# msracver/Relation-Networks-for-Object-Detection

Measured on AMD Instinct MI355X. Metric: images/sec (1000x600, 300 ROIs), higher is better.
Workload: dtype bf16

## Files before the change

include/relnet_hip.h:

```cpp
#ifndef RELNET_HIP_H
#define RELNET_HIP_H

#ifdef __cplusplus
extern "C" {
#endif

enum { RELNET_F32 = 0, RELNET_BF16 = 1 };

int relnet_version(void);
const char* relnet_last_error(void);
unsigned long long relnet_stream_capture_id(void* stream);

void _nms(int* keep_out, int* num_out, const float* boxes_host, int boxes_num, int boxes_dim,
          float nms_overlap_thresh, int device_id);

int relnet_proposal_decode(const float* cls_prob, const long* cls_strides4, const float* deltas,
                           const long* delta_strides4, const float* im_info, const double* base_anchors,
                           float* boxes , float* scores , int B, int A, int h, int w,
                           int feat_stride, int min_size, int softmax_pairs, void* stream);
int relnet_topk_sort(const float* scores, const float* boxes, float* out_boxes5, int* out_index,
                     int* out_count, int B, int n, int K, void* stream);
int relnet_nms_mask(const float* boxes5, const int* counts , unsigned long long* mask,
                    int B, int n, int n_stride, float thresh, void* stream);
int relnet_nms_scan(const unsigned long long* mask, const float* boxes5, const int* counts, float* rois,
// ... 73 lines not shown

int relnet_geometry_bias(const float* boxes, int box_stride, int box_off, const float* wp_t, const float* bp,
                         const float* divisors8, void* bias, int bias_half , float* pos_mat,
                         float* pos_emb, int B, int N, int M, int Mpad, int fc_dim, int nmod, void* stream);

int relnet_relation_attention(const void* q, long q_ld, long q_bs, const void* k, long k_ld, long k_bs,
                              const void* vwt, long vwt_ld, long vwt_bs, const void* bias, int bias_half,
                              long bias_bs, const float* bout, const void* resid, long resid_ld, long resid_bs, void* out,
                              long out_ld, long out_bs, void* out_act, long act_ld, long act_bs, float* logits,
                              int B, int H, int N, int M, int Mpad, float scale, int in_dtype, int out_dtype,
                              void* stream);

int relnet_relation_attention_kc(const void* q, long q_ld, long q_bs, const void* k, long k_ld, long k_bs,
                                 const void* vwt, long vwt_ld, long vwt_bs, const void* bias, int bias_half,
                                 long bias_bs, const float* bout, const void* resid, long resid_ld, long resid_bs, void* out,
                                 long out_ld, long out_bs, void* out_act, long act_ld, long act_bs, float* logits,
                                 int B, int H, int N, int M, int Mpad, float scale, int in_dtype, int out_dtype,
                                 const int* key_count, void* stream);
void relnet_relation_attention_debug_lds_f32(int on);

int relnet_relation_attention_fused(const void* q, long q_ld, long q_bs, const void* k, long k_ld, long k_bs,
                                    const void* vwt, long vwt_ld, long vwt_bs, const float* boxes, int box_stride,
                                    int box_off, const float* wp, const float* bp, const float* divisors8,
                                    const float* bout, const void* resid, long resid_ld, long resid_bs, void* out,
                                    long out_ld, long out_bs, void* out_act, long act_ld, long act_bs, int B, int H,
                                    int N, int M, int Mpad, float scale, void* stream);

int relnet_bottleneck_chain(const void* mid2, const void* x, const void* w3f, const void* w1f, const float* b3,
                            const float* b1, void* x_next, void* mid1_next, long P, int mid, void* stream);
int relnet_bottleneck_chain_proj(const void* mid2, const void* x_in, const void* w3f, const void* wpf, const void* w1f,
                                 const float* b3p, const float* b1, void* x_next, void* mid1_next, long P, int mid, void* stream);
int relnet_bottleneck_chain_s2(const void* mid2, const void* x, const void* w3f, const float* b3, void* x_next, int B, int H,
                               int W, int mid, void* stream);

int relnet_conv3x3_c64(const void* in, const void* w_frag, const float* bias, int relu, void* out, int B, int H, int W,
                       void* stream);
int relnet_conv3x3_c64_s2(const void* in, const void* w_frag, const float* bias, int relu, void* out, int B, int H, int W,
                          void* stream);


int relnet_pack_w_frag(const void* w, long ldw, void* out, int N, int K, void* stream);
int relnet_conv2d_nhwc_wf(const void* in, long in_pix, long in_img, const void* w, const void* w_frag, const float* bias,
                          const void* resid, int relu, void* out, long ldc, int B, int H, int W, int Cin, int Cout, int R,
                          int S, int stride, int dil, int pad, int out_dtype, void* stream);

int relnet_detect_head(const float* cls_score, long cs_ld, const float* bbox_pred, long bp_ld, const float* rois,
                       const float* im_info, float* cls_prob, double* boxes, int R, int C, int rois_per_image,
                       int delta_off, void* stream);
int relnet_detect_head_ex(const float* cls_score, long cs_ld, const float* bbox_pred, long bp_ld, const float* rois,
                          const float* im_info, float* cls_prob, double* boxes, int R, int C, int rois_per_image,
                          int delta_off, const int* n_valid, void* stream);
int relnet_class_nms(const float* cls_prob, const double* boxes, double* dets, int* counts, int B, int N, int C,
                     float score_thresh, double nms_param, int soft, int max_picks, void* stream);
int relnet_class_nms_ex(const float* cls_prob, const double* scores64, const double* boxes, double* dets, int* counts,
                        int* pick_index, int B, int N, int C, float score_thresh, double nms_param, int soft,
                        int max_picks, void* stream);
int relnet_class_nms_hist_bins(void);
int relnet_class_nms_topk(const float* cls_prob, const double* boxes, double* dets, int* counts, void* hist, int B, int N, int C,
                          float score_thresh, double nms_param, int soft, int max_picks, int top_k, void* stream);
int relnet_image_topk(const double* dets, const int* counts, double* thresh, int* total, float* out,
                      int* out_count, int B, int NC, int N, int max_per_image, int max_out, void* stream);

int relnet_lnms_prepare(const float* cls_score, long cs_ld, const float* bbox_pred, long bp_ld, const float* rois,
                        const float* im_info, float* prob , float* boxes , int B, int N,
                        int C, int delta_off, const float* means4, const float* stds4, void* stream);
int relnet_lnms_prepare_ex(const float* cls_score, long cs_ld, const float* bbox_pred, long bp_ld, const float* rois,
// ... 214 lines not shown
```

relation-networks-for-object-detection_amd/backbone.py:

```python
import math
import os

import torch
import torch.nn.functional as F

from . import ops

UNITS = (3, 4, 23, 3)
FILTERS = (256, 512, 1024, 2048)
EPS = 1e-5
PIXEL_MEANS = (103.06, 115.90, 123.15)


def unit_names(fpn=False):
    out = []
    in_ch = 64
    for si, (n, oc) in enumerate(zip(UNITS, FILTERS)):
        stage = si + 2
        for u in range(n):
            if n <= 3 or stage == 2 or stage == 5:
                name = 'abc'[u]
            else:
                name = 'a' if u == 0 else 'b%d' % u
            stride = 2 if (u == 0 and (stage in (3, 4) or (fpn and stage == 5))) else 1
# ... 51 lines not shown
        p['res5%s_branch2b_offset_weight' % u] = nrm(dcn_offset_std, 72, 512, 3, 3)
        p['res5%s_branch2b_offset_bias' % u] = torch.zeros(72)
    p['offset_weight'] = nrm(dcn_offset_std, 98, 256 * 49); p['offset_bias'] = torch.zeros(98)
    if fpn:
        for lvl, cin in ((32, 2048), (16, 1024), (8, 512), (4, 256)):
            p['fpn_ft%d_1x1_weight' % lvl] = nrm(0.01, 256, cin, 1, 1); p['fpn_ft%d_1x1_bias' % lvl] = torch.zeros(256)
            p['fpn_ft%d_3x3_weight' % lvl] = nrm(0.01, 256, 256, 3, 3); p['fpn_ft%d_3x3_bias' % lvl] = torch.zeros(256)
        p['fpn_ft64_3x3_weight'] = nrm(0.01, 256, 256, 3, 3); p['fpn_ft64_3x3_bias'] = torch.zeros(256)
        p['roi_pool_fc1_weight'] = nrm(0.01, 1024, 256 * 49); p['roi_pool_fc1_bias'] = torch.zeros(1024)
        p['roi_pool_fc2_weight'] = nrm(0.01, 1024, 1024); p['roi_pool_fc2_bias'] = torch.zeros(1024)
    return p


def fold_bn(w, gamma, beta, mean, var, eps=EPS):
    s = gamma.double() / torch.sqrt(var.double() + eps)
    return (w.double() * s.view(-1, 1, 1, 1)).float(), (beta.double() - mean.double() * s).float()


class Backbone(object):

    def __init__(self, params, dtype=torch.bfloat16, device='cuda', channels_last=True, impl=None, stem='hip', dcn=False,
                 fpn=False, chain=True, frozen_only=False, pixel_means=PIXEL_MEANS):
        self.dtype, self.device, self.dcn, self.fpn = dtype, device, dcn, fpn
        self.frozen_only = frozen_only
        self.pixel_means = tuple(float(v) for v in pixel_means)
        self.use_chain = chain
        env = os.environ.get('RELNET_STAGE_SPLIT')
        if env not in (None, '', '0'):
            self.stage_split = {int(a): int(b) for a, b in (kv.split(':') for kv in env.split(','))}
        if os.environ.get('RELNET_INPLACE_EXPAND') is not None:
            self.inplace_expand = os.environ['RELNET_INPLACE_EXPAND'] not in ('', '0')
        if os.environ.get('RELNET_QUARTER_UNITS') is not None:
            self.quarter_units = os.environ['RELNET_QUARTER_UNITS'] not in ('', '0')
        self.impl = impl or ('hip' if dtype == torch.bfloat16 else ('hip32' if dtype == torch.float32 and torch.device(device).type == 'cuda' else 'miopen'))
        if self.impl == 'hip' and torch.device(device).type == 'cuda':
            ops.asm_selfcheck()
        self.stem = stem
        assert self.impl in ('hip', 'hip32', 'miopen') and (self.impl != 'hip' or dtype == torch.bfloat16) and (self.impl != 'hip32' or dtype == torch.float32)
        self.mf = torch.channels_last if channels_last else torch.contiguous_format
        self.w = {}
        self.wp = {}
        self.wf = {}
        self.b32 = {}
        self.wp32 = {}
        for conv, bn, oc, ic, k in conv_bn_names():
            if frozen_only and not conv.startswith(('conv1', 'res2')):
                continue
            w, b = fold_bn(params[conv + '_weight'], params[bn + '_gamma'], params[bn + '_beta'],
                           params[bn + '_moving_mean'], params[bn + '_moving_var'])
            self._put(conv, w, b)
        if frozen_only:
            pass
        elif fpn:
            for lvl in (32, 16, 8, 4):
                for k in ('1x1', '3x3'):
                    name = 'fpn_ft%d_%s' % (lvl, k)
                    self._put(name, params[name + '_weight'], params[name + '_bias'])
        else:
            for name in ('rpn_conv_3x3', 'rpn_cls_score', 'rpn_bbox_pred', 'conv_new_1'):
                self._put(name, params[name + '_weight'], params[name + '_bias'])
            self._put('rpn_out', torch.cat([params['rpn_cls_score_weight'], params['rpn_bbox_pred_weight']], 0),
                      torch.cat([params['rpn_cls_score_bias'], params['rpn_bbox_pred_bias']], 0))
        self.units = [u for u in unit_names(fpn) if not frozen_only or u[0] == 2]
        self.wp_dcn = {}
        if dcn and not frozen_only:
            for u in 'abc':
                name = 'res5%s_branch2b' % u
                self._put(name + '_offset', params[name + '_offset_weight'], params[name + '_offset_bias'])
                w, b = fold_bn(params[name + '_weight'], params['bn5%s_branch2b_gamma' % u], params['bn5%s_branch2b_beta' % u],
                               params['bn5%s_branch2b_moving_mean' % u], params['bn5%s_branch2b_moving_var' % u])
                self.wp_dcn[name] = (ops.pack_conv_weight(w, self.dtype, self.device), b.to(self.device, torch.float32).contiguous())
        if self.impl == 'hip':
            w1, b1 = fold_bn(params['conv1_weight'], params['bn_conv1_gamma'], params['bn_conv1_beta'],
                             params['bn_conv1_moving_mean'], params['bn_conv1_moving_var'])
            self.w_stem = ops.pack_stem_weight(w1, self.dtype, self.device)
            self.zero_bias64 = torch.zeros(64, device=self.device, dtype=torch.float32)
        self.chain, self.halo3, self.chain_proj = {}, {}, {}
        if self.impl == 'hip' and chain:
            reduce_mids = tuple(m for m in ops.CHAIN_MIDS if m != 256 or os.environ.get('RELNET_CHAIN_REDUCE256', '1') != '0')
            for (st, nm, ic, mc, oc, stride, dil, proj), nxt in zip(self.units, self.units[1:] + [None]):
                if nxt is not None and nxt[0] == st and not nxt[7] and mc in reduce_mids:
                    w3, b3, _ = self.wp['res%s_branch2c' % nm]
                    w1n, b1n, _ = self.wp['res%s_branch2a' % nxt[1]]
                    self.chain[nm] = (ops.pack_w_frag(w3), ops.pack_chain_w1(w1n), b3, b1n)
                elif mc in ops.CHAIN_EXPAND_MIDS:
                    w3, b3, _ = self.wp['res%s_branch2c' % nm]
                    self.chain[nm] = (ops.pack_w_frag(w3), None, b3, None)
            for (st, nm, ic, mc, oc, stride, dil, proj) in self.units:
                if proj and stride == 1 and mc == 64 and ic == 64 and nm in self.chain:
                    w3f, w1f, b3, b1n = self.chain[nm]
                    wp_, bp_, _ = self.wp['res%s_branch1' % nm]
                    self.chain_proj[nm] = (w3f, ops.pack_w_frag(wp_), w1f, (b3 + bp_).contiguous(), b1n)
            for st, nm, ic, mc, oc, stride, dil, proj in self.units:
                if mc in ops.HALO3_CHANNELS and dil == 1 and not (self.dcn and st == 5):
                    w, b, _ = self.wp['res%s_branch2b' % nm]
                    self.halo3['res%s_branch2b' % nm] = (ops.pack_w_frag(w, panel_only=False), b)

    def _put(self, name, w, b):
        self.w[name] = (w.to(self.device, self.dtype).contiguous(memory_format=self.mf),
                        b.to(self.device, self.dtype))
        if self.impl == 'hip':
            self.b32[name] = b.to(self.device, torch.float32).contiguous()
        if self.impl == 'hip32':
            if w.shape[1] % 16:
                wz = torch.zeros((w.shape[0], (w.shape[1] + 15) // 16 * 16) + tuple(w.shape[2:]), dtype=w.dtype)
                wz[:, :w.shape[1]] = w
                w = wz
            self.wp32[name] = (ops.pack_conv_weight(w, torch.float32, self.device), b.to(self.device, torch.float32).contiguous(), int(w.shape[2]))
        if self.impl == 'hip' and w.shape[1] % 64 == 0:
            self.wp[name] = (ops.pack_conv_weight(w, self.dtype, self.device),
                             b.to(self.device, torch.float32).contiguous(), int(w.shape[2]))
            if self.dtype == torch.bfloat16 and tuple(w.shape[1:]) == (256, 1, 1) and w.shape[0] % 256 == 0 \
                    and name.endswith('_branch2c'):
                self.wf[name] = ops.pack_w_frag(self.wp[name][0])

    def _hconv(self, x, name, stride=1, pad=0, dil=1, relu=False, resid=None, out_dtype=None):
        w, b, k = self.wp[name]
        return ops.conv2d_nhwc(x, w, b, ksize=k, stride=stride, pad=pad, dil=dil, relu=relu, resid=resid,
                               out_dtype=out_dtype, w_frag=self.wf.get(name))

    def _float_image(self, data, im_info, dtype):
        if data.dtype != torch.uint8:
            return data
        return ops.image_transform_u8(data, self.pixel_means, im_info, dtype=dtype)

    def forward_res2(self, data, im_info=None):
        if self.impl == 'hip32':
            assert self.frozen_only
            return self._forward_hip32(self._float_image(data, im_info, torch.float32))
        x = ops.stem_fused(data, self.w_stem, self.b32['conv1'], im_info, self.pixel_means)
        y_next = None
        self.last_chain_units = []
        for unit in self.units:
            if unit[0] != 2:
                break
            x, y_next = self._unit_hip(x, unit, y_next)
        return x

    def _forward_hip(self, data, rpn_hook=None, im_info=None):
        if self.stem == 'hip':
            x = ops.stem_fused(data, self.w_stem, self.b32['conv1'], im_info, self.pixel_means)
        elif self.stem == 'hip3':
            x = ops.stem_conv7(self._float_image(data, im_info, torch.float32), self.w_stem, self.b32['conv1'], relu=True)
            x = ops.stem_bias_relu_pool(x, self.zero_bias64)
        else:
            x = self._float_image(data, im_info, torch.float32).to(self.dtype).contiguous(memory_format=self.mf)
            x = F.conv2d(x, self.w['conv1'][0], None, stride=2, padding=3)
            x = ops.stem_bias_relu_pool(x.permute(0, 2, 3, 1), self.b32['conv1'])
        conv4 = None
        ends = {}
        y_next = None
        side, hooked = None, None
        self.last_chain_units, self.last_side_stream, self.last_stage_split = [], False, {}
        self.last_quarter_units = []
        compact = False
        ui = 0
        while ui < len(self.units):
            unit = self.units[ui]
            stage, proj = unit[0], unit[7]
            if stage == 5 and conv4 is None:
                conv4 = x
                if rpn_hook is not None and not self.fpn:
                    main = torch.cuda.current_stream()
                    side = self._side_stream()
                    self.last_side_stream = True
                    side.wait_stream(main)
                    with torch.cuda.stream(side):
                        hooked = self._rpn_head(conv4)
                        hooked = hooked + (rpn_hook(hooked[0], hooked[1]),)
            if proj and stage > 2:
                ends[stage - 1] = x
            nsplit = self._stage_split(stage, x, unit) if proj else 1
            if nsplit > 1:
                stage_units = [u for u in self.units if u[0] == stage]
                x = self._run_stage_split(x, stage_units, nsplit)
                ui += len(stage_units)
                continue
            quarter = self._quarter_ok(x, unit, self.units[ui + 1] if ui + 1 < len(self.units) else None)
            x, y_next = self._unit_hip(x, unit, y_next, inplace=self.inplace_expand, quarter=quarter, subsampled=compact)
            compact = quarter
            ui += 1
        conv5 = x
        nchw = lambda t: t.permute(0, 3, 1, 2)
        if self.fpn:
            tops = {32: self._hconv(conv5, 'fpn_ft32_1x1')}
            for lvl, src in ((16, ends[4]), (8, ends[3]), (4, ends[2])):
                tops[lvl] = ops.upsample2x_add_(self._hconv(src, 'fpn_ft%d_1x1' % lvl), tops[lvl * 2])
            out = {'fpn_ft%d' % lvl: nchw(self._hconv(tops[lvl], 'fpn_ft%d_3x3' % lvl, pad=1)) for lvl in (4, 8, 16, 32)}
            out.update(conv4=nchw(conv4), conv5=nchw(conv5))
            return out
        feat = self._hconv(conv5, 'conv_new_1', relu=True)
        out = dict(conv4=nchw(conv4), conv5=nchw(conv5), conv_new_1_relu=nchw(feat))
        if hooked is not None:
            torch.cuda.current_stream().wait_stream(side)
            out.update(rpn_cls_score=hooked[0], rpn_bbox_pred=hooked[1], rpn_hook=hooked[2])
        else:
            out['rpn_cls_score'], out['rpn_bbox_pred'] = self._rpn_head(conv4)
        return out

    stage_split = None
    inplace_expand = True

    quarter_units = True

    def _quarter_ok(self, x, unit, nxt):
        stage, nm, ic, mc, oc, stride, dil, proj = unit
        if not self.quarter_units or self.fpn or nxt is None or nxt[0] != stage + 1 or nxt[5] != 2 or not nxt[7]:
            return False
        ch = self.chain.get(nm)
        if ch is None or ch[1] is not None or mc not in ops.CHAIN_S2_MIDS or proj or dil != 1 or (self.dcn and stage == 5):
            return False
        if mc in ops.HALO3_CHANNELS and ('res%s_branch2b' % nm) not in self.halo3:
            return False
        if self.stage_split and (self._stage_split(stage, x, unit) > 1 or self._stage_split(nxt[0], x, nxt) > 1):
            return False
        B, H, W, C = x.shape
        return C == oc and x.numel() * 2 < (1 << 32) and ops.chain_worthwhile(B * ((H - 1) // 2 + 1) * ((W - 1) // 2 + 1), mc)

    def _stage_split(self, stage, x, unit):
        return int(self.stage_split.get(stage, 1)) if self.stage_split else 1

    def _run_stage_split(self, x, stage_units, nsplit):
        B = x.shape[0]
        stage = stage_units[0][0]
        st, nm, ic, mc, oc, stride, dil, proj = stage_units[0]
        Ho, Wo = (x.shape[1] - 1) // stride + 1, (x.shape[2] - 1) // stride + 1
        out = torch.empty((B, Ho, Wo, oc), device=x.device, dtype=x.dtype)
        bounds = [(B * i) // nsplit for i in range(nsplit + 1)]
        self.last_stage_split[stage] = [hi - lo for lo, hi in zip(bounds, bounds[1:])]
        for lo, hi in zip(bounds, bounds[1:]):
            xs, ys = x[lo:hi], None
            for unit in stage_units:
                xs, ys = self._unit_hip(xs, unit, ys, sc_out=out[lo:hi] if unit[7] else None, inplace=self.inplace_expand, force_chain=True)
            if xs.data_ptr() != out[lo:hi].data_ptr():
                out[lo:hi].copy_(xs)
        return out

    def _unit_hip(self, x, unit, y_pre=None, sc_out=None, inplace=False, force_chain=False, quarter=False, subsampled=False):
        stage, nm, ic, mc, oc, stride, dil, proj = unit
        if subsampled:
            assert stride == 2 and proj
            stride = 1
        if quarter:
            y = y_pre if y_pre is not None else self._hconv(x, 'res%s_branch2a' % nm, relu=True)
            if ('res%s_branch2b' % nm) in self.halo3:
                y = ops.conv3x3_halo_s2(y.contiguous(), *self.halo3['res%s_branch2b' % nm], relu=True)
            else:
                y = self._hconv(y, 'res%s_branch2b' % nm, stride=2, pad=1, relu=True)
            w3f, _, b3, _ = self.chain[nm]
            if nm not in self.last_chain_units:
                self.last_chain_units.append(nm)
            self.last_quarter_units.append(nm)
            return ops.bottleneck_chain_s2(y, x.contiguous(), w3f, b3), None
        fuse_proj = (nm in self.chain_proj and sc_out is None and x.is_contiguous()
                     and (force_chain or ops.chain_worthwhile(x.numel() // x.shape[-1], mc)))
        if fuse_proj:
            sc = None
        elif proj:
            w, b, k = self.wp['res%s_branch1' % nm]
            sc = ops.conv2d_nhwc(x, w, b, ksize=k, stride=stride, out=sc_out)
        else:
            sc = x
        y = y_pre if y_pre is not None else self._hconv(x, 'res%s_branch2a' % nm, stride=stride, relu=True)
        if self.dcn and stage == 5:
            y = self._deform_2b(y.permute(0, 3, 1, 2), 'res%s_branch2b' % nm,
                                self._hconv(y, 'res%s_branch2b_offset' % nm, pad=2, dil=2, out_dtype=torch.float32).permute(0, 3, 1, 2))
            y = y.permute(0, 2, 3, 1)
        elif ('res%s_branch2b' % nm) in self.halo3:
            y = ops.conv3x3_halo(y.contiguous(), *self.halo3['res%s_branch2b' % nm], relu=True)
        else:
            y = self._hconv(y, 'res%s_branch2b' % nm, pad=dil, dil=dil, relu=True)
        if fuse_proj:
            if nm not in self.last_chain_units:
                self.last_chain_units.append(nm)
            return ops.bottleneck_chain_proj(y, x, *self.chain_proj[nm])
        ch = self.chain.get(nm)
        if ch is not None and not force_chain and not ops.chain_worthwhile(y.numel() // y.shape[-1], y.shape[-1]):
            ch = None
        if ch is not None:
            if nm not in self.last_chain_units:
                self.last_chain_units.append(nm)
            return ops.bottleneck_chain(y, sc.contiguous(), *ch, inplace=inplace and sc.is_contiguous())
        return self._hconv(y, 'res%s_branch2c' % nm, relu=True, resid=sc), None

    def _rpn_head(self, conv4):
        r = self._hconv(conv4, 'rpn_conv_3x3', pad=1, relu=True)
        rpn = self._hconv(r, 'rpn_out', out_dtype=torch.float32)
        na2 = self.w['rpn_cls_score'][0].shape[0]
        return rpn[..., :na2].permute(0, 3, 1, 2), rpn[..., na2:].permute(0, 3, 1, 2)

# ... 95 lines not shown
```

relation-networks-for-object-detection_amd/csrc/bottleneck.hip:

```cpp
#include "common.h"

namespace relnet {

typedef const __attribute__((address_space(1))) void* gas_ptr;
typedef __attribute__((address_space(3))) void* las_ptr;

__device__ __forceinline__ void chain_glds16(const void* src, unsigned lds_byte_addr) {
  asm volatile("s_mov_b32 m0, %1\n\ts_nop 0\n\tglobal_load_lds_dwordx4 %0, off" ::"v"(src), "s"(lds_byte_addr) : "memory", "m0");
}

struct ChainArgs {
  const unsigned short* m2;
  const unsigned short* x;
  const uint4* w3f;
  const uint4* w1f;
  const float* b3;
  const float* b1;
  const unsigned short* xin;
  const uint4* wpf;
  unsigned short* xn;
  unsigned short* m1;
  int P;
  int H, W, Ho, Wo;
  int dbg;
// ... 170 lines not shown
      asm volatile("s_waitcnt lgkmcnt(0)" ::: "memory");
      __builtin_amdgcn_wave_barrier();
      if constexpr (PROJ) { flush(p0, p); __builtin_amdgcn_wave_barrier(); }
    }
    if constexpr (!PROJ) flush(p0, NP - 1);
    if constexpr (!REDUCE) continue;
    unsigned char* sb = stage + (PROJ ? 0 : ((NP - 1) & 1) * 4096);
#pragma unroll
    for (int hc = 0; hc < RT / 2; ++hc) {
#pragma unroll
      for (int r2 = 0; r2 < 2; ++r2)
#pragma unroll
        for (int g = 0; g < 4; ++g) {
          const int rt = 2 * hc + r2;
          const float4 bv = *(const float4*)(sB1 + rt * 32 + 8 * g + 4 * half);
          const float v0 = fmaxf(m1acc[rt][4 * g + 0] + bv.x, 0.f), v1 = fmaxf(m1acc[rt][4 * g + 1] + bv.y, 0.f);
          const float v2 = fmaxf(m1acc[rt][4 * g + 2] + bv.z, 0.f), v3 = fmaxf(m1acc[rt][4 * g + 3] + bv.w, 0.f);
          *(uint2*)(sb + l31 * 128 + (((r2 * 4 + g) ^ ((l31 >> 1) & 7)) << 4) + 8 * half) = make_uint2(pack_bf16x2(v0, v1), pack_bf16x2(v2, v3));
        }
      asm volatile("s_waitcnt lgkmcnt(0)" ::: "memory");
      __builtin_amdgcn_wave_barrier();
      const unsigned char* sl = sb + lane * 16;
      const uint4 v0 = *(const uint4*)sl, v1 = *(const uint4*)(sl + 1024), v2 = *(const uint4*)(sl + 2048), v3 = *(const uint4*)(sl + 3072);
      asm volatile("s_waitcnt lgkmcnt(0)" ::: "memory");
      auto put = [&](int i, const uint4& v) {
        const int row = 8 * i + drow;
        if (p0 + row < a.P) *(uint4*)(a.m1 + (long)(p0 + row) * MID + hc * 64 + ((dslot ^ ((row >> 1) & 7)) << 3)) = v;
      };
      put(0, v0); put(1, v1); put(2, v2); put(3, v3);
    }
  }
}




constexpr int kRolesLdsBytes = 2 * 32768 + 4 * 4 * 4096 + 4 * 4096 + (1024 + 256) * 4;
__global__ __launch_bounds__(512) void chain256_roles_kernel(ChainArgs a) {
  constexpr int MID = 256, COUT = 4 * MID, KS = MID / 16, RT = MID / 32, NP = COUT / 64, NSTEP = 2 * NP, NTL = 4, NBUF = 4;
  constexpr int W3P = KS * 1024, W1P = 2 * RT * 1024, SLOT = W3P + W1P, WBYTES = 2 * SLOT;
  constexpr int STG = NBUF * 4096, M1S = WBYTES + NTL * STG, BIAS = M1S + NTL * 4096;
  static_assert(BIAS + (COUT + MID) * 4 == kRolesLdsBytes, "host launch and kernel disagree on the LDS layout");
  extern __shared__ __attribute__((aligned(16))) unsigned char smem[];
  const int tid = threadIdx.x, lane = tid & 63;
  const int wave = __builtin_amdgcn_readfirstlane(tid >> 6);
  const int half = lane >> 5, l31 = lane & 31, drow = lane >> 3, dslot = lane & 7;
  const unsigned lds0 = (unsigned)(unsigned long)(las_ptr)smem;
  float* sB3 = (float*)(smem + BIAS);
  float* sB1 = sB3 + COUT;
  for (int i = tid; i < COUT; i += 512) sB3[i] = a.b3[i];
  for (int i = tid; i < MID; i += 512) sB1[i] = a.b1[i];
  const int ntile = (a.P + 31) / 32, nset = (ntile + NTL - 1) / NTL;
  const int n_iter = (nset - (int)blockIdx.x + (int)gridDim.x - 1) / (int)gridDim.x;
  if (n_iter <= 0) return;
  const int G = n_iter * NSTEP, NPASS = n_iter * NP;
  auto tile_p0 = [&](int it, int T) { return (((int)blockIdx.x + it * (int)gridDim.x) * NTL + T) * 32; };
  auto issue_x = [&](int T, int Pg) {
    if (a.dbg & 4) return;
    const int p0 = tile_p0(Pg / NP, T), p = Pg % NP;
    unsigned char* sb = smem + WBYTES + T * STG + (Pg % NBUF) * 4096;
#pragma unroll
    for (int i = 0; i < 4; ++i) {
      const int row = 8 * i + drow;
      const unsigned off = ((unsigned)min(p0 + row, a.P - 1) * COUT + p * 64 + ((dslot ^ ((row >> 1) & 7)) << 3)) * 2u;
      chain_glds16((const unsigned char*)a.x + off, __builtin_amdgcn_readfirstlane(lds0 + (unsigned)(sb - smem) + i * 1024));
    }
  };
  auto issue_w = [&](int g, int l) {
// ... 223 lines not shown
  const long ntile = (P + 31) / 32;
  const unsigned grid = (unsigned)(ntile < 8 * 256 ? (ntile + 7) / 8 : 256);
  const size_t lds = 65536 + 65536 + (size_t)5 * mid * 4;
  if (mid == 64) bottleneck_chain_kernel<64, false, false, 1, false, true><<<grid, 512, lds, (hipStream_t)stream>>>(a);
  else bottleneck_chain_kernel<128, true, false, 1, false, true><<<grid, 512, lds, (hipStream_t)stream>>>(a);
  return check_launch("relnet_bottleneck_chain_s2");
}

extern "C" int relnet_bottleneck_chain_proj(const void* mid2, const void* x_in, const void* w3f, const void* wpf, const void* w1f,
                                            const float* b3p, const float* b1, void* x_next, void* mid1_next, long P, int mid,
                                            void* stream) {
  RELNET_REQUIRE(mid2 && x_in && w3f && wpf && b3p && x_next, "relnet_bottleneck_chain_proj: null operand");
  RELNET_REQUIRE((w1f && b1 && mid1_next) || (!w1f && !b1 && !mid1_next), "relnet_bottleneck_chain_proj: w1f, b1 and mid1_next are given together (or all NULL)");
  RELNET_REQUIRE(mid == 64, "relnet_bottleneck_chain_proj: mid = %d unsupported (64)", mid);
  RELNET_REQUIRE(P > 0 && P * 8 * mid < (1L << 32), "relnet_bottleneck_chain_proj: bad pixel count %ld (x_next is addressed with 32-bit byte offsets: the 4 mid-channel map must stay below 4 GiB)", P);
  ChainArgs a;
  a.m2 = (const unsigned short*)mid2; a.x = nullptr; a.w3f = (const uint4*)w3f; a.w1f = (const uint4*)w1f;
  a.b3 = b3p; a.b1 = b1; a.xn = (unsigned short*)x_next; a.m1 = (unsigned short*)mid1_next; a.P = (int)P;
  a.xin = (const unsigned short*)x_in; a.wpf = (const uint4*)wpf; a.dbg = 0;
  a.H = a.W = a.Ho = a.Wo = 0;
  static relnet::PerDeviceOnce attr_once;
  if (attr_once.first()) {
    hipFuncSetAttribute((const void*)bottleneck_chain_kernel<64, false, true, 1, true>, hipFuncAttributeMaxDynamicSharedMemorySize, 160 * 1024);
    hipFuncSetAttribute((const void*)bottleneck_chain_kernel<64, false, false, 1, true>, hipFuncAttributeMaxDynamicSharedMemorySize, 160 * 1024);
  }
  const long ntile = (P + 31) / 32;
  const unsigned grid = (unsigned)(ntile < 8 * 256 ? (ntile + 7) / 8 : 256);
  const size_t lds = (size_t)4 * (8192 + 8192 + (mid1_next ? 8192 : 0)) + 8 * 4096 + (size_t)5 * mid * 4;
  if (mid1_next) bottleneck_chain_kernel<64, false, true, 1, true><<<grid, 512, lds, (hipStream_t)stream>>>(a);
  else bottleneck_chain_kernel<64, false, false, 1, true><<<grid, 512, lds, (hipStream_t)stream>>>(a);
  return check_launch("relnet_bottleneck_chain_proj");
}

namespace relnet {

__device__ __attribute__((aligned(16))) const unsigned int g_zero_chunk[4] = {0u, 0u, 0u, 0u};

struct Halo3Args {
  const unsigned short* in;
  const uint4* wf;
  const float* bias;
  unsigned short* out;
  int B, H, W, relu;
  int tiles_x, tiles_y;
  int Ho, Wo;
};

constexpr int kHaloW = 34, kHaloSlots = 40;
constexpr int kHaloBytes = 10 * kHaloSlots * 128;
constexpr int kHalo2Row = 65, kHalo2Even = 33;
constexpr int kHalo2Dma = (9 * kHalo2Row + 7) / 8;
constexpr int kHalo2Bytes = kHalo2Dma * 1024;

template <bool S2>
__global__ __launch_bounds__(512) void conv3x3_c64_halo_kernel(Halo3Args a) {
  constexpr int NR = S2 ? 1 : 2;
  constexpr int HB = S2 ? kHalo2Bytes : kHaloBytes;
  extern __shared__ __attribute__((aligned(16))) unsigned char smem[];
  unsigned char* sOutDense = smem + 2 * HB;
  const int tid = threadIdx.x, lane = tid & 63;
  const int wave = __builtin_amdgcn_readfirstlane(tid >> 6);
  const int half = lane >> 5, l31 = lane & 31;
  const int chh = wave & 1, rg = wave >> 1;
  bf16x8 wfrag[36];
#pragma unroll
  for (int ks = 0; ks < 36; ++ks) wfrag[ks] = *(const bf16x8*)&a.wf[(chh * 36 + ks) * 64 + lane];
// ... 153 lines not shown
```

relation-networks-for-object-detection_amd/lib.py:

```python
import ctypes as C
import os
import sys

HERE = os.path.dirname(os.path.abspath(__file__))
LIB_PATH = os.environ.get('RELNET_LIB') or os.path.join(HERE, 'librelnet_hip.so')

F32, BF16 = 0, 1


class RelnetError(RuntimeError):
    pass


_lib = None

_vp, _i, _l, _f, _d = C.c_void_p, C.c_int, C.c_long, C.c_float, C.c_double

_SIGNATURES = {
    'relnet_version': (C.c_int, []),
    'relnet_last_error': (C.c_char_p, []),
    'relnet_gemm_nt': (C.c_int, [_vp, _l, _l, _vp, _l, _l, _vp, _l, _l, _vp, _i, _vp, _i,
                                 _i, _i, _i, _i, _i, _i, _vp]),
    'relnet_geometry_bias': (C.c_int, [_vp, _i, _i, _vp, _vp, _vp, _vp, _i, _vp, _vp, _i, _i, _i, _i,
                                       _i, _i, _vp]),
    'relnet_relation_attention': (C.c_int, [_vp, _l, _l, _vp, _l, _l, _vp, _l, _l, _vp, _i, _l, _vp,
                                            _vp, _l, _l, _vp, _l, _l, _vp, _l, _l, _vp,
                                            _i, _i, _i, _i, _i, _f, _i, _i, _vp]),
    'relnet_relation_attention_kc': (C.c_int, [_vp, _l, _l, _vp, _l, _l, _vp, _l, _l, _vp, _i, _l, _vp,
                                               _vp, _l, _l, _vp, _l, _l, _vp, _l, _l, _vp,
                                               _i, _i, _i, _i, _i, _f, _i, _i, _vp, _vp]),
    'relnet_relation_attention_fused': (C.c_int, [_vp, _l, _l, _vp, _l, _l, _vp, _l, _l, _vp, _i, _i, _vp, _vp, _vp,
                                                  _vp, _vp, _l, _l, _vp, _l, _l, _vp, _l, _l,
                                                  _i, _i, _i, _i, _i, _f, _vp]),
    'relnet_bottleneck_chain': (C.c_int, [_vp, _vp, _vp, _vp, _vp, _vp, _vp, _vp, _l, _i, _vp]),
    'relnet_bottleneck_chain_proj': (C.c_int, [_vp, _vp, _vp, _vp, _vp, _vp, _vp, _vp, _vp, _l, _i, _vp]),
    'relnet_conv3x3_c64': (C.c_int, [_vp, _vp, _vp, _i, _vp, _i, _i, _i, _vp]),
    'relnet_conv3x3_c64_s2': (C.c_int, [_vp, _vp, _vp, _i, _vp, _i, _i, _i, _vp]),
    'relnet_bottleneck_chain_s2': (C.c_int, [_vp, _vp, _vp, _vp, _vp, _i, _i, _i, _i, _vp]),
    'relnet_proposal_decode': (C.c_int, [_vp, _vp, _vp, _vp, _vp, _vp, _vp, _vp, _i, _i, _i, _i, _i, _i, _i, _vp]),
    'relnet_topk_sort': (C.c_int, [_vp, _vp, _vp, _vp, _vp, _i, _i, _i, _vp]),
    'relnet_nms_mask': (C.c_int, [_vp, _vp, _vp, _i, _i, _i, _f, _vp]),
    'relnet_nms_scan': (C.c_int, [_vp, _vp, _vp, _vp, _vp, _vp, _vp, _i, _i, _i, _i, _i, _i, _vp]),
    '_nms': (None, [_vp, _vp, _vp, _i, _i, _f, _i]),
    'relnet_roi_pool_fwd': (C.c_int, [_vp, _vp, _vp, _vp, _vp, _vp, _i, _i, _i, _i, _i, _i, _f, _i, _i, _vp]),
    'relnet_roi_align_fwd': (C.c_int, [_vp, _vp, _vp, _vp, _vp, _i, _i, _i, _i, _i, _i, _f, _i, _i, _i, _i, _vp]),
    'relnet_roi_align_bwd': (C.c_int, [_vp, _vp, _vp, _vp, _vp, _i, _i, _i, _i, _i, _i, _f, _i, _i, _i, _i, _vp]),
    'relnet_roi_align_levels_fwd': (C.c_int, [_vp, _vp, _vp, _vp, _vp, _i, _vp, _vp, _vp, _vp] + [_i] * 9 + [_vp]),
    'relnet_roi_align_levels_bwd': (C.c_int, [_vp, _vp, _vp, _vp, _vp, _vp, _vp, _vp, _vp] + [_i] * 10 + [_vp]),
    'relnet_roi_pool_bwd': (C.c_int, [_vp, _vp, _vp, _vp, _vp, _l, _l, _i, _i, _i, _i, _i, _i, _i, _vp]),
    'relnet_roi_pool_bwd_ex': (C.c_int, [_vp, _vp, _vp, _vp, _vp, _l, _l, _l, _i, _i, _i, _i, _i, _i, _i, _vp]),
    'relnet_roi_pool_fpn_bwd_ex': (C.c_int, [_vp, _vp, _vp, _vp, _vp, _vp, _vp, _vp, _vp, _i, _i, _i, _i, _i, _i, _i, _vp]),
    'relnet_detect_head': (C.c_int, [_vp, _l, _vp, _l, _vp, _vp, _vp, _vp, _i, _i, _i, _i, _vp]),
    'relnet_detect_head_ex': (C.c_int, [_vp, _l, _vp, _l, _vp, _vp, _vp, _vp, _i, _i, _i, _i, _vp, _vp]),
    'relnet_class_nms': (C.c_int, [_vp, _vp, _vp, _vp, _i, _i, _i, _f, C.c_double, _i, _i, _vp]),
    'relnet_class_nms_ex': (C.c_int, [_vp, _vp, _vp, _vp, _vp, _vp, _i, _i, _i, _f, C.c_double, _i, _i, _vp]),
    'relnet_class_nms_topk': (C.c_int, [_vp, _vp, _vp, _vp, _vp, _i, _i, _i, _f, C.c_double, _i, _i, _i, _vp]),
    'relnet_class_nms_hist_bins': (C.c_int, []),
    'relnet_bbox_overlaps': (C.c_int, [_vp, _vp, _vp, _i, _i, _vp]),
    'relnet_image_topk': (C.c_int, [_vp, _vp, _vp, _vp, _vp, _vp, _i, _i, _i, _i, _i, _vp]),
    'relnet_conv2d_nhwc': (C.c_int, [_vp, _l, _l, _vp, _vp, _vp, _i, _vp, _l, _i, _i, _i, _i, _i, _i, _i, _i, _i, _i, _i, _vp]),
    'relnet_conv2d_nhwc_f32': (C.c_int, [_vp, _l, _l, _vp, _vp, _vp, _i, _vp, _l, _i, _i, _i, _i, _i, _i, _i, _i, _i, _i, _vp]),
    'relnet_maxpool_nhwc_f32': (C.c_int, [_vp, _vp, _i, _i, _i, _i, _i, _i, _vp]),
    'relnet_pack_w_frag': (C.c_int, [_vp, _l, _vp, _i, _i, _vp]),
    'relnet_conv2d_nhwc_wf': (C.c_int, [_vp, _l, _l, _vp, _vp, _vp, _vp, _i, _vp, _l, _i, _i, _i, _i, _i, _i, _i, _i, _i, _i, _i, _vp]),
    'relnet_deformable_im2col': (C.c_int, [_vp, _vp, _vp, _vp, _vp, _l] + [_i] * 15 + [_vp]),
    'relnet_deformable_psroi_pool_fwd': (C.c_int, [_vp, _vp, _vp, _vp, _vp, _vp, _vp] + [_i] * 9 + [_f, _f, _i, _i, _i, _vp]),
    'relnet_roi_pool_fpn_fwd': (C.c_int, [_vp, _vp, _vp, _vp, _vp, _i, _vp, _vp, _vp, _vp, _vp, _i, _i, _i, _i, _i, _i, _vp]),
    'relnet_fpn_roi_dispatch': (C.c_int, [_vp, _i, _i, _vp, _vp, _vp, _vp, _i, _i, _i, _vp]),
    'relnet_fpn_roi_dispatch_ex': (C.c_int, [_vp, _i, _i, _vp, _vp, _vp, _vp, _i, _i, _i, _vp, _i, _i, _vp, _vp]),
    'relnet_upsample2x_add': (C.c_int, [_vp, _vp, _i, _i, _i, _i, _i, _vp]),
    'relnet_softmax_output': (C.c_int, [_vp, _vp, _vp, _vp, _vp, _l, _i, _l, _i, _f, _f, _vp]),
# ... 149 lines not shown
```

relation-networks-for-object-detection_amd/ops.py:

```python
import math
import os

import torch

from . import lib as _lib

F32, BF16 = _lib.F32, _lib.BF16


def _dt(t):
    if t.dtype == torch.float32:
        return F32
    if t.dtype == torch.bfloat16:
        return BF16
    raise TypeError("unsupported dtype %s (float32 or bfloat16)" % t.dtype)


def _chk(*ts):
    for t in ts:
        if t is not None:
            if not t.is_cuda:
                raise _lib.RelnetError("relnet ops need GPU tensors (HIP kernels only; no CPU fallback)")


# ... 578 lines not shown
    m1 = torch.empty_like(mid2) if w1_frag is not None else None
    _lib.call('relnet_bottleneck_chain', mid2.data_ptr(), x.data_ptr(), w3_frag.data_ptr(), _ptr(w1_frag), b3.data_ptr(),
              _ptr(b1), xn.data_ptr(), _ptr(m1), mid2.numel() // mid, mid, _stream())
    return xn, m1


CHAIN_S2_MIDS = (64, 128)


def bottleneck_chain_s2(mid2, x, w3_frag, b3):
    _chk(mid2, x, w3_frag, b3)
    mid = mid2.shape[-1]
    B, H, W, C = x.shape
    assert mid in CHAIN_S2_MIDS and C == 4 * mid and mid2.shape == (B, (H - 1) // 2 + 1, (W - 1) // 2 + 1, mid)
    assert mid2.is_contiguous() and x.is_contiguous() and x.numel() * 2 < (1 << 32)
    assert mid2.dtype == torch.bfloat16 and x.dtype == torch.bfloat16 and b3.dtype == torch.float32
    xn = torch.empty(mid2.shape[:-1] + (C,), device=x.device, dtype=x.dtype)
    _lib.call('relnet_bottleneck_chain_s2', mid2.data_ptr(), x.data_ptr(), w3_frag.data_ptr(), b3.data_ptr(), xn.data_ptr(), B, H, W, mid,
              _stream())
    return xn


def bottleneck_chain_proj(mid2, x_in, w3_frag, wp_frag, w1_frag, b3p, b1):
    _chk(mid2, x_in, w3_frag, wp_frag, w1_frag, b3p, b1)
    mid = mid2.shape[-1]
    assert mid == 64 and x_in.shape == mid2.shape and mid2.is_contiguous() and x_in.is_contiguous()
    assert mid2.dtype == torch.bfloat16 and x_in.dtype == torch.bfloat16 and b3p.dtype == torch.float32
    assert (w1_frag is None) == (b1 is None)
    xn = torch.empty(mid2.shape[:-1] + (4 * mid,), device=mid2.device, dtype=torch.bfloat16)
    m1 = torch.empty_like(mid2) if w1_frag is not None else None
    _lib.call('relnet_bottleneck_chain_proj', mid2.data_ptr(), x_in.data_ptr(), w3_frag.data_ptr(), wp_frag.data_ptr(), _ptr(w1_frag),
              b3p.data_ptr(), _ptr(b1), xn.data_ptr(), _ptr(m1), mid2.numel() // mid, mid, _stream())
    return xn, m1


def conv2d_nhwc(x, w_packed, bias, ksize=1, stride=1, pad=0, dil=1, relu=False, resid=None, out=None,
                out_dtype=None, w_frag=None):
    _chk(x, w_packed, bias, resid, out)
    if x.dtype == torch.float32:
        return conv2d_nhwc_f32(x, w_packed, bias, ksize, stride, pad, dil, relu, resid, out)
    assert x.dtype == torch.bfloat16 and w_packed.dtype == torch.bfloat16 and x.stride(3) == 1
    B, H, W, Cin = x.shape
    assert x.stride(1) == W * x.stride(2), "rows of an image must be dense in W"
    Cout = w_packed.shape[0]
    assert w_packed.shape[1] == ksize * ksize * Cin and w_packed.is_contiguous()
    Hout = (H + 2 * pad - dil * (ksize - 1) - 1) // stride + 1
    Wout = (W + 2 * pad - dil * (ksize - 1) - 1) // stride + 1
    odt = out_dtype or (out.dtype if out is not None else x.dtype)
    if out is None:
        out = torch.empty((B, Hout, Wout, Cout), device=x.device, dtype=odt)
    assert out.shape == (B, Hout, Wout, Cout) and out.stride(3) == 1
    assert out.stride(1) == Wout * out.stride(2) and out.stride(0) == Hout * out.stride(1)
    if resid is not None:
        assert resid.dtype == out.dtype and resid.stride() == out.stride()
    gemm_workspace()
    _lib.call('relnet_conv2d_nhwc_wf', x.data_ptr(), x.stride(2), x.stride(0), w_packed.data_ptr(), _ptr(w_frag), _ptr(bias),
              _ptr(resid), int(relu), out.data_ptr(), out.stride(2), B, H, W, Cin, Cout, ksize, ksize,
              stride, dil, pad, _dt(out), _stream(),
              tag='M%d_N%d_K%d_k%d' % (B * Hout * Wout, Cout, ksize * ksize * Cin, ksize))
    return out


def conv2d_nhwc_f32(x, w_packed, bias, ksize=1, stride=1, pad=0, dil=1, relu=False, resid=None, out=None):
    _chk(x, w_packed, bias, resid, out)
    assert x.dtype == torch.float32 and w_packed.dtype == torch.float32 and x.stride(3) == 1
    B, H, W, Cin = x.shape
# ... 732 lines not shown
```

Measured before the change: 2956.

## Fuse stage-entry projection and reduce 1x1 convs into one kernel

```diff
diff --git a/include/relnet_hip.h b/include/relnet_hip.h
--- a/include/relnet_hip.h
+++ b/include/relnet_hip.h
@@ -129,6 +129,8 @@
                                  const float* b3p, const float* b1, void* x_next, void* mid1_next, long P, int mid, void* stream);
 int relnet_bottleneck_chain_s2(const void* mid2, const void* x, const void* w3f, const float* b3, void* x_next, int B, int H,
                                int W, int mid, void* stream);
+int relnet_stage_entry(const void* x, const void* wf, const float* bias, void* out_proj, void* out_red, long P, int kin,
+                       int n_proj, int n_red, void* stream);
 
 int relnet_conv3x3_c64(const void* in, const void* w_frag, const float* bias, int relu, void* out, int B, int H, int W,
                        void* stream);
diff --git a/relation-networks-for-object-detection_amd/backbone.py b/relation-networks-for-object-detection_amd/backbone.py
--- a/relation-networks-for-object-detection_amd/backbone.py
+++ b/relation-networks-for-object-detection_amd/backbone.py
@@ -107,6 +107,8 @@
             self.inplace_expand = os.environ['RELNET_INPLACE_EXPAND'] not in ('', '0')
         if os.environ.get('RELNET_QUARTER_UNITS') is not None:
             self.quarter_units = os.environ['RELNET_QUARTER_UNITS'] not in ('', '0')
+        if os.environ.get('RELNET_ENTRY_UNITS') is not None:
+            self.entry_units = os.environ['RELNET_ENTRY_UNITS'] not in ('', '0')
         self.impl = impl or ('hip' if dtype == torch.bfloat16 else ('hip32' if dtype == torch.float32 and torch.device(device).type == 'cuda' else 'miopen'))
         if self.impl == 'hip' and torch.device(device).type == 'cuda':
             ops.asm_selfcheck()
@@ -150,7 +152,7 @@
                              params['bn_conv1_moving_mean'], params['bn_conv1_moving_var'])
             self.w_stem = ops.pack_stem_weight(w1, self.dtype, self.device)
             self.zero_bias64 = torch.zeros(64, device=self.device, dtype=torch.float32)
-        self.chain, self.halo3, self.chain_proj = {}, {}, {}
+        self.chain, self.halo3, self.chain_proj, self.entry = {}, {}, {}, {}
         if self.impl == 'hip' and chain:
             reduce_mids = tuple(m for m in ops.CHAIN_MIDS if m != 256 or os.environ.get('RELNET_CHAIN_REDUCE256', '1') != '0')
             for (st, nm, ic, mc, oc, stride, dil, proj), nxt in zip(self.units, self.units[1:] + [None]):
@@ -166,6 +168,12 @@
                     w3f, w1f, b3, b1n = self.chain[nm]
                     wp_, bp_, _ = self.wp['res%s_branch1' % nm]
                     self.chain_proj[nm] = (w3f, ops.pack_w_frag(wp_), w1f, (b3 + bp_).contiguous(), b1n)
+            for (st, nm, ic, mc, oc, stride, dil, proj) in self.units:
+                if proj and ic in ops.ENTRY_KINS and oc % 64 == 0 and mc % 64 == 0 and nm not in self.chain_proj \
+                        and not (self.dcn and st == 5):
+                    wp_, bp_, _ = self.wp['res%s_branch1' % nm]
+                    w1_, b1_, _ = self.wp['res%s_branch2a' % nm]
+                    self.entry[nm] = ops.pack_stage_entry(wp_, bp_, w1_, b1_) + (oc,)
             for st, nm, ic, mc, oc, stride, dil, proj in self.units:
                 if mc in ops.HALO3_CHANNELS and dil == 1 and not (self.dcn and st == 5):
                     w, b, _ = self.wp['res%s_branch2b' % nm]
@@ -227,7 +235,7 @@
         y_next = None
         side, hooked = None, None
         self.last_chain_units, self.last_side_stream, self.last_stage_split = [], False, {}
-        self.last_quarter_units = []
+        self.last_quarter_units, self.last_entry_units = [], []
         compact = False
         ui = 0
         while ui < len(self.units):
@@ -278,6 +286,8 @@
 
     quarter_units = True
 
+    entry_units = True
+
     def _quarter_ok(self, x, unit, nxt):
         stage, nm, ic, mc, oc, stride, dil, proj = unit
         if not self.quarter_units or self.fpn or nxt is None or nxt[0] != stage + 1 or nxt[5] != 2 or not nxt[7]:
@@ -331,6 +341,10 @@
                      and (force_chain or ops.chain_worthwhile(x.numel() // x.shape[-1], mc)))
         if fuse_proj:
             sc = None
+        elif (proj and stride == 1 and nm in self.entry and y_pre is None and sc_out is None and x.is_contiguous()
+              and self.entry_units and ops.entry_worthwhile(x.numel() // x.shape[-1], ic)):
+            sc, y_pre = ops.stage_entry(x, *self.entry[nm])
+            self.last_entry_units.append(nm)
         elif proj:
             w, b, k = self.wp['res%s_branch1' % nm]
             sc = ops.conv2d_nhwc(x, w, b, ksize=k, stride=stride, out=sc_out)
diff --git a/relation-networks-for-object-detection_amd/csrc/bottleneck.hip b/relation-networks-for-object-detection_amd/csrc/bottleneck.hip
--- a/relation-networks-for-object-detection_amd/csrc/bottleneck.hip
+++ b/relation-networks-for-object-detection_amd/csrc/bottleneck.hip
@@ -226,8 +226,118 @@
   }
 }
 
-
-
+struct EntryArgs {
+  const unsigned short* x;
+  const uint4* wf;
+  const float* bias;
+  unsigned short* sc;
+  unsigned short* m1;
+  int P, n_proj, n_red;
+};
+
+template <int KIN, int KSPLIT, int TPW>
+__global__ __launch_bounds__(512) void stage_entry_kernel(EntryArgs a) {
+  constexpr int KS = KIN / 16, KSS = KS / KSPLIT;
+  constexpr int SLOT = 2 * KSS * 1024, STG = 4096;
+  static_assert(SLOT == 32768, "a ring slot is 32 KiB: four LDS-DMA instructions per wave and step");
+  extern __shared__ __attribute__((aligned(16))) unsigned char smem[];
+  const int tid = threadIdx.x, lane = tid & 63;
+  const int wave = __builtin_amdgcn_readfirstlane(tid >> 6);
+  const int half = lane >> 5, l31 = lane & 31;
+  unsigned char* stage = smem + 2 * SLOT + wave * (TPW * STG);
+  float* sB = (float*)(smem + 2 * SLOT + 8 * TPW * STG);
+  const int NP = (a.n_proj + a.n_red) >> 6, npp = a.n_proj >> 6, nstep = NP * KSPLIT;
+  for (int i = tid; i < NP * 64; i += 512) sB[i] = a.bias[i];
+  __syncthreads();
+  const int ntile = (a.P + 31) / 32;
+  const int drow = lane >> 3, dslot = lane & 7;
+  auto issue_w = [&](int st, int slot) {
+    const int p = st / KSPLIT, kh = st % KSPLIT;
+    unsigned char* wb = smem + slot * SLOT;
+#pragma unroll
+    for (int i = 0; i < 4; ++i) {
+      const int q = wave + 8 * i, ct = q / KSS, ks = q % KSS;
+      __builtin_amdgcn_global_load_lds((gas_ptr)(a.wf + ((long)((p * 2 + ct) * KS + kh * KSS + ks) * 64 + lane)), (las_ptr)(wb + q * 1024), 16, 0, 0);
+    }
+  };
+  auto flush = [&](int p0, int p, int j) {
+    const unsigned char* sb = stage + j * STG + lane * 16;
+    const uint4 v0 = *(const uint4*)sb, v1 = *(const uint4*)(sb + 1024), v2 = *(const uint4*)(sb + 2048), v3 = *(const uint4*)(sb + 3072);
+    asm volatile("s_waitcnt lgkmcnt(0)" ::: "memory");
+    const bool red = p >= npp;
+    unsigned char* ob = red ? (unsigned char*)a.m1 : (unsigned char*)a.sc;
+    const unsigned ld = red ? (unsigned)a.n_red : (unsigned)a.n_proj, c0 = (unsigned)(red ? p - npp : p) * 64u;
+    auto put = [&](int i, const uint4& v) {
+      const int row = 8 * i + drow;
+      if (p0 + row < a.P) *(uint4*)(ob + ((unsigned)(p0 + row) * ld + c0 + ((dslot ^ ((row >> 1) & 7)) << 3)) * 2u) = v;
+    };
+    put(0, v0); put(1, v1); put(2, v2); put(3, v3);
+  };
+
+  const int t_first = (blockIdx.x * 8 + wave) * TPW;
+  const int t_step = gridDim.x * 8 * TPW;
+  const int n_iter = ((ntile + 8 * TPW - 1) / (8 * TPW) - (int)blockIdx.x + (int)gridDim.x - 1) / (int)gridDim.x;
+  if (n_iter <= 0) return;
+  int gs = 0;
+  issue_w(0, 0);
+  for (int it = 0; it < n_iter; ++it) {
+    const int p0 = (t_first + it * t_step) * 32;
+    bf16x8 xf[TPW][KS];
+#pragma unroll
+    for (int j = 0; j < TPW; ++j) {
+      const int px = min(p0 + 32 * j + l31, a.P - 1);
+#pragma unroll
+      for (int ks = 0; ks < KS; ++ks) xf[j][ks] = *(const bf16x8*)((const unsigned char*)a.x + ((unsigned)px * KIN + 16 * ks + 8 * half) * 2u);
+    }
+#pragma unroll 1
+    for (int p = 0; p < NP; ++p) {
+      f32x16 acc[TPW][2];
+#pragma unroll
+      for (int kh = 0; kh < KSPLIT; ++kh) {
+        const int st = p * KSPLIT + kh;
+        asm volatile("s_waitcnt vmcnt(0)\n\ts_barrier" ::: "memory");
+        if (kh == 0 && p > 0)
+#pragma unroll
+          for (int j = 0; j < TPW; ++j) flush(p0 + 32 * j, p - 1, j);
+        if (st + 1 < nstep) issue_w(st + 1, (gs + 1) & 1);
+        else if (it + 1 < n_iter) issue_w(0, (gs + 1) & 1);
+        const uint4* w = (const uint4*)(smem + (gs & 1) * SLOT);
+        ++gs;
+#pragma unroll
+        for (int ct = 0; ct < 2; ++ct) {
+          if (kh == 0)
+#pragma unroll
+            for (int j = 0; j < TPW; ++j)
+#pragma unroll
+              for (int r = 0; r < 16; ++r) acc[j][ct][r] = 0.f;
+#pragma unroll
+          for (int ks = 0; ks < KSS; ++ks) {
+            const bf16x8 wv = *(const bf16x8*)&w[(ct * KSS + ks) * 64 + lane];
+#pragma unroll
+            for (int j = 0; j < TPW; ++j) acc[j][ct] = __builtin_amdgcn_mfma_f32_32x32x16_bf16(wv, xf[j][kh * KSS + ks], acc[j][ct], 0, 0, 0);
+          }
+        }
+      }
+      const bool relu = p >= npp;
+#pragma unroll
+      for (int j = 0; j < TPW; ++j)
+#pragma unroll
+        for (int ct = 0; ct < 2; ++ct) {
+#pragma unroll
+          for (int g = 0; g < 4; ++g) {
+            const float4 bv = *(const float4*)(sB + p * 64 + ct * 32 + 8 * g + 4 * half);
+            float v0 = acc[j][ct][4 * g + 0] + bv.x, v1 = acc[j][ct][4 * g + 1] + bv.y, v2 = acc[j][ct][4 * g + 2] + bv.z, v3 = acc[j][ct][4 * g + 3] + bv.w;
+            if (relu) { v0 = fmaxf(v0, 0.f); v1 = fmaxf(v1, 0.f); v2 = fmaxf(v2, 0.f); v3 = fmaxf(v3, 0.f); }
+            *(uint2*)(stage + j * STG + l31 * 128 + (((ct * 4 + g) ^ ((l31 >> 1) & 7)) << 4) + 8 * half) = make_uint2(pack_bf16x2(v0, v1), pack_bf16x2(v2, v3));
+          }
+        }
+      asm volatile("s_waitcnt lgkmcnt(0)" ::: "memory");
+      __builtin_amdgcn_wave_barrier();
+    }
+#pragma unroll
+    for (int j = 0; j < TPW; ++j) flush(p0 + 32 * j, NP - 1, j);
+  }
+}
 
 constexpr int kRolesLdsBytes = 2 * 32768 + 4 * 4 * 4096 + 4 * 4096 + (1024 + 256) * 4;
 __global__ __launch_bounds__(512) void chain256_roles_kernel(ChainArgs a) {
@@ -517,6 +627,29 @@
   return check_launch("relnet_bottleneck_chain_proj");
 }
 
+extern "C" int relnet_stage_entry(const void* x, const void* wf, const float* bias, void* out_proj, void* out_red, long P, int kin,
+                                  int n_proj, int n_red, void* stream) {
+  RELNET_REQUIRE(x && wf && bias && out_proj && out_red, "relnet_stage_entry: null operand");
+  RELNET_REQUIRE(kin == 256, "relnet_stage_entry: kin = %d unsupported (256)", kin);
+  RELNET_REQUIRE(n_proj > 0 && n_red > 0 && n_proj % 64 == 0 && n_red % 64 == 0 && n_proj + n_red <= 4096,
+                 "relnet_stage_entry: n_proj = %d, n_red = %d (both must be positive multiples of 64, at most 4096 together)", n_proj, n_red);
+  RELNET_REQUIRE(P > 0 && P * (kin > n_proj ? kin : n_proj) * 2 < (1L << 32) && P * n_red * 2 < (1L << 32),
+                 "relnet_stage_entry: bad pixel count %ld (x and both outputs are addressed with 32-bit byte offsets: each must stay below 4 GiB)", P);
+  relnet::EntryArgs a;
+  a.x = (const unsigned short*)x; a.wf = (const uint4*)wf; a.bias = bias;
+  a.sc = (unsigned short*)out_proj; a.m1 = (unsigned short*)out_red; a.P = (int)P; a.n_proj = n_proj; a.n_red = n_red;
+  static relnet::PerDeviceOnce attr_once;
+  if (attr_once.first()) {
+    hipFuncSetAttribute((const void*)relnet::stage_entry_kernel<256, 1, 2>, hipFuncAttributeMaxDynamicSharedMemorySize, 160 * 1024);
+  }
+  const int tpw = 2;
+  const long nset = ((P + 31) / 32 + 8 * tpw - 1) / (8 * tpw);
+  const unsigned grid = (unsigned)(nset < 256 ? nset : 256);
+  const size_t lds = 65536  + (size_t)8 * tpw * 4096  + (size_t)(n_proj + n_red) * 4;
+  relnet::stage_entry_kernel<256, 1, 2><<<grid, 512, lds, (hipStream_t)stream>>>(a);
+  return check_launch("relnet_stage_entry");
+}
+
 namespace relnet {
 
 __device__ __attribute__((aligned(16))) const unsigned int g_zero_chunk[4] = {0u, 0u, 0u, 0u};
diff --git a/relation-networks-for-object-detection_amd/lib.py b/relation-networks-for-object-detection_amd/lib.py
--- a/relation-networks-for-object-detection_amd/lib.py
+++ b/relation-networks-for-object-detection_amd/lib.py
@@ -37,6 +37,7 @@
     'relnet_conv3x3_c64': (C.c_int, [_vp, _vp, _vp, _i, _vp, _i, _i, _i, _vp]),
     'relnet_conv3x3_c64_s2': (C.c_int, [_vp, _vp, _vp, _i, _vp, _i, _i, _i, _vp]),
     'relnet_bottleneck_chain_s2': (C.c_int, [_vp, _vp, _vp, _vp, _vp, _i, _i, _i, _i, _vp]),
+    'relnet_stage_entry': (C.c_int, [_vp, _vp, _vp, _vp, _vp, _l, _i, _i, _i, _vp]),
     'relnet_proposal_decode': (C.c_int, [_vp, _vp, _vp, _vp, _vp, _vp, _vp, _vp, _i, _i, _i, _i, _i, _i, _i, _vp]),
     'relnet_topk_sort': (C.c_int, [_vp, _vp, _vp, _vp, _vp, _i, _i, _i, _vp]),
     'relnet_nms_mask': (C.c_int, [_vp, _vp, _vp, _i, _i, _i, _f, _vp]),
diff --git a/relation-networks-for-object-detection_amd/ops.py b/relation-networks-for-object-detection_amd/ops.py
--- a/relation-networks-for-object-detection_amd/ops.py
+++ b/relation-networks-for-object-detection_amd/ops.py
@@ -634,6 +634,39 @@
     _lib.call('relnet_bottleneck_chain_proj', mid2.data_ptr(), x_in.data_ptr(), w3_frag.data_ptr(), wp_frag.data_ptr(), _ptr(w1_frag),
               b3p.data_ptr(), _ptr(b1), xn.data_ptr(), _ptr(m1), mid2.numel() // mid, mid, _stream())
     return xn, m1
+
+
+ENTRY_KINS = (256,)
+ENTRY_MIN_PIXELS = {256: 196608}
+
+
+def entry_worthwhile(pixels, kin):
+    return kin in ENTRY_MIN_PIXELS and pixels >= ENTRY_MIN_PIXELS[kin] and pixels * 4 * kin < (1 << 32)
+
+
+def pack_stage_entry(wp, bp, w1, b1):
+    _chk(wp, bp, w1, b1)
+    assert wp.shape[1] == w1.shape[1] and wp.shape[0] % 64 == 0 and w1.shape[0] % 64 == 0
+    return (pack_w_frag(torch.cat([wp, w1], 0).contiguous(), panel_only=False),
+            torch.cat([bp.to(torch.float32), b1.to(torch.float32)]).contiguous())
+
+
+def stage_entry(x, w_frag, bias, n_proj, out=None):
+    _chk(x, w_frag, bias)
+    B, H, W, kin = x.shape
+    n_red = bias.numel() - n_proj
+    assert kin in ENTRY_KINS and x.is_contiguous() and x.dtype == torch.bfloat16
+    assert w_frag.dtype == torch.bfloat16 and w_frag.is_contiguous() and bias.dtype == torch.float32 and bias.is_contiguous()
+    assert n_proj > 0 and n_red > 0 and n_proj % 64 == 0 and n_red % 64 == 0 and w_frag.numel() == (n_proj + n_red) * kin
+    if out is None:
+        out = (torch.empty((B, H, W, n_proj), device=x.device, dtype=x.dtype), torch.empty((B, H, W, n_red), device=x.device, dtype=x.dtype))
+    sc, m1 = out
+    _chk(sc, m1)
+    assert sc.shape == (B, H, W, n_proj) and m1.shape == (B, H, W, n_red) and sc.is_contiguous() and m1.is_contiguous()
+    assert sc.dtype == torch.bfloat16 and m1.dtype == torch.bfloat16
+    _lib.call('relnet_stage_entry', x.data_ptr(), w_frag.data_ptr(), bias.data_ptr(), sc.data_ptr(), m1.data_ptr(), B * H * W, kin,
+              n_proj, n_red, _stream())
+    return sc, m1
 
 
 def conv2d_nhwc(x, w_packed, bias, ksize=1, stride=1, pad=0, dil=1, relu=False, resid=None, out=None,
```

Result: no change. 2940 (-0.5%).
